# 236088/reflect-sampling-nerf

Hardware: AMD Instinct MI355X
Metric: rays/sec (train step) at 4096 rays x 128 samples, 1/2/4/8 MI355X; PSNR vs ref (higher is better)
Workload: dtype f32

## Files before the change

### reflect_sampling_nerf_amd/csrc/rsn_epilogues.h

```cpp
#pragma once
#include "rsn_gemm_loops.h"

template <int NBO>
__device__ __forceinline__ void init_acc(f32x16 (&acc)[NBO], const float* __restrict__ bias, int h) {
#pragma unroll
  for (int nb = 0; nb < NBO; ++nb)
#pragma unroll
    for (int q = 0; q < 4; ++q) {
      const float4 bv = *reinterpret_cast<const float4*>(bias + nb * 32 + 8 * q + 4 * h);
      acc[nb][4 * q + 0] = bv.x;
      acc[nb][4 * q + 1] = bv.y;
      acc[nb][4 * q + 2] = bv.z;
      acc[nb][4 * q + 3] = bv.w;
    }
}

template <int NBO>
__device__ __forceinline__ void zero_acc(f32x16 (&acc)[NBO]) {
#pragma unroll
  for (int nb = 0; nb < NBO; ++nb)
#pragma unroll
    for (int r = 0; r < 16; ++r) acc[nb][r] = 0.0f;
}

template <int NBO>
__device__ __forceinline__ void zero_acc16(f32x4 (&acc)[NBO][2][2]) {
#pragma unroll
  for (int nb = 0; nb < NBO; ++nb)
#pragma unroll
    for (int q = 0; q < 4; ++q) acc[nb][q >> 1][q & 1] = f32x4{0.0f, 0.0f, 0.0f, 0.0f};
}

template <int Q>
__device__ __forceinline__ unsigned relu_bits4q(unsigned b, const float4 v) {
  const unsigned lo[4] = {__float_as_uint(v.x), __float_as_uint(v.y), __float_as_uint(v.z), __float_as_uint(v.w)};
#pragma unroll
  for (int t = 0; t < 4; ++t) {
    unsigned bit, nb;
    if (Q == 0 && t == 0) {
      asm("v_min_u32 %0, %1, 1" : "=v"(bit) : "v"(lo[t]));
      b = bit;
    } else if (t == 0) {
      asm("v_min_u32 %0, %2, 1\n\tv_lshl_or_b32 %1, %0, %3, %4" : "=&v"(bit), "=v"(nb) : "v"(lo[t]), "n"(4 * Q), "v"(b));
      b = nb;
    } else if (t == 1) {
      asm("v_min_u32 %0, %2, 1\n\tv_lshl_or_b32 %1, %0, %3, %4" : "=&v"(bit), "=v"(nb) : "v"(lo[t]), "n"(4 * Q + 1), "v"(b));
      b = nb;
    } else if (t == 2) {
      asm("v_min_u32 %0, %2, 1\n\tv_lshl_or_b32 %1, %0, %3, %4" : "=&v"(bit), "=v"(nb) : "v"(lo[t]), "n"(4 * Q + 2), "v"(b));
      b = nb;
    } else {
      asm("v_min_u32 %0, %2, 1\n\tv_lshl_or_b32 %1, %0, %3, %4" : "=&v"(bit), "=v"(nb) : "v"(lo[t]), "n"(4 * Q + 3), "v"(b));
      b = nb;
    }
  }
  return b;
}
__device__ __forceinline__ unsigned relu_bits4(unsigned b, const float4 v, int q) {
  return q == 0 ? relu_bits4q<0>(b, v) : (q == 1 ? relu_bits4q<1>(b, v) : (q == 2 ? relu_bits4q<2>(b, v) : relu_bits4q<3>(b, v)));
}

template <int NBO>
struct ReluBits {
  unsigned w[NBO / 2];
};

template <int NBO>
__device__ __forceinline__ ReluBits<NBO> load_relu_bits(const unsigned* __restrict__ bits) {
  ReluBits<NBO> m;
  if (NBO >= 8) {
#pragma unroll
    for (int w4 = 0; w4 < NBO / 8; ++w4) {
      const uint4 v = *reinterpret_cast<const uint4*>(bits + w4 * 4);
      m.w[w4 * 4 + 0] = v.x; m.w[w4 * 4 + 1] = v.y; m.w[w4 * 4 + 2] = v.z; m.w[w4 * 4 + 3] = v.w;
    }
  } else {
#pragma unroll
    for (int w = 0; w < NBO / 2; ++w) m.w[w] = bits[w];
  }
  return m;
}

__device__ __forceinline__ unsigned bit_mask(int word, int pos) {
  unsigned m;
  asm("v_bfe_i32 %0, %1, %2, 1" : "=v"(m) : "v"(word), "n"(pos));
  return m;
}

template <int NBO, bool SBF = false, class SV = float*>
__device__ __forceinline__ void store_masked_bits(const f32x16 (&acc)[NBO], float4* xl, const ReluBits<NBO>& m, int h,
                                                  SV save = nullptr) {
#pragma unroll
  for (int nb = 0; nb < NBO; ++nb)
#pragma unroll
    for (int q = 0; q < 4; ++q) {
      const int word = m.w[nb / 2];
      const int base = (nb & 1) * 16 + 4 * q;
      float4 v;
      v.x = __uint_as_float(__float_as_uint(acc[nb][4 * q + 0]) & bit_mask(word, base + 0));
      v.y = __uint_as_float(__float_as_uint(acc[nb][4 * q + 1]) & bit_mask(word, base + 1));
      v.z = __uint_as_float(__float_as_uint(acc[nb][4 * q + 2]) & bit_mask(word, base + 2));
      v.w = __uint_as_float(__float_as_uint(acc[nb][4 * q + 3]) & bit_mask(word, base + 3));
      xl[(nb * 4 + q) * 64] = v;
      if (sv_on(save)) sv_put<SBF>(save, nb, q, h, v);
    }
}

template <int NBO>
__device__ __forceinline__ void store_masked_bits16(const f32x4 (&acc)[NBO][2][2], float4* xl, const ReluBits<NBO> (&m)[2], int lane) {
  const Lane16 g = lane16(lane);
  float4* xs = xl - lane + g.ol + g.kh * 64;
#pragma unroll
  for (int ph = 0; ph < 2; ++ph)
#pragma unroll
    for (int nb = 0; nb < NBO; ++nb) {
      const int word = (int)(m[ph].w[nb / 2] >> (4 * g.kh));
#pragma unroll
      for (int rh = 0; rh < 2; ++rh) {
        const int base = (nb & 1) * 16 + 8 * rh;
        const f32x4& a = acc[nb][rh][ph];
        float4 v;
        v.x = __uint_as_float(__float_as_uint(a[0]) & bit_mask(word, base + 0));
        v.y = __uint_as_float(__float_as_uint(a[1]) & bit_mask(word, base + 1));
        v.z = __uint_as_float(__float_as_uint(a[2]) & bit_mask(word, base + 2));
        v.w = __uint_as_float(__float_as_uint(a[3]) & bit_mask(word, base + 3));
        xs[(nb * 4 + 2 * rh) * 64 + 16 * ph] = v;
      }
    }
}

template <int NBO>
__device__ __forceinline__ void store_act16(const f32x4 (&acc)[NBO][2][2], float4* xl, int lane) {
  const Lane16 g = lane16(lane);
  float4* xs = xl - lane + g.ol + g.kh * 64;
#pragma unroll
  for (int nb = 0; nb < NBO; ++nb)
#pragma unroll
    for (int q = 0; q < 4; ++q) {
      const f32x4& a = acc[nb][q >> 1][q & 1];
      xs[(nb * 4 + 2 * (q >> 1)) * 64 + 16 * (q & 1)] = make_float4(a[0], a[1], a[2], a[3]);
    }
}

template <int NBS, bool RELU, bool SBF, bool REINIT, class ACC, class SV>
__device__ __forceinline__ void store_act_body(ACC& acc, float4* xl, SV save, int h, const float* __restrict__ bias, unsigned* bits) {
  unsigned bw[NBS / 2 > 0 ? NBS / 2 : 1];
#pragma unroll
  for (int nb = 0; nb < NBS; ++nb) {
    unsigned b16 = 0u;
#pragma unroll
    for (int q = 0; q < 4; ++q) {
      float4 v = make_float4(acc[nb][4 * q + 0], acc[nb][4 * q + 1], acc[nb][4 * q + 2], acc[nb][4 * q + 3]);
      if (RELU) {
        v.x = relu_f(v.x);
        v.y = relu_f(v.y);
        v.z = relu_f(v.z);
        v.w = relu_f(v.w);
        b16 = relu_bits4(b16, v, q);
      }
      xl[(nb * 4 + q) * 64] = v;
      if (sv_on(save)) sv_put<SBF>(save, nb, q, h, v);
      if constexpr (REINIT) {
        const float4 bv = *reinterpret_cast<const float4*>(bias + nb * 32 + 8 * q + 4 * h);
        acc[nb][4 * q + 0] = bv.x;
        acc[nb][4 * q + 1] = bv.y;
        acc[nb][4 * q + 2] = bv.z;
        acc[nb][4 * q + 3] = bv.w;
      }
    }
    if (RELU) {
      if (nb & 1) bw[nb / 2] |= b16 << 16; else bw[nb / 2] = b16;
    }
  }
  if (RELU && bits) {
    if (NBS >= 8) {
#pragma unroll
      for (int w4 = 0; w4 < NBS / 8; ++w4)
        *reinterpret_cast<uint4*>(bits + w4 * 4) = make_uint4(bw[w4 * 4], bw[w4 * 4 + 1], bw[w4 * 4 + 2], bw[w4 * 4 + 3]);
    } else {
#pragma unroll
      for (int w = 0; w < NBS / 2; ++w) bits[w] = bw[w];
    }
  }
}
template <int NBO, int NBS, bool RELU, bool SBF = false, class SV = float*>
__device__ __forceinline__ void store_act(const f32x16 (&acc)[NBO], float4* xl, SV save = nullptr, int h = 0,
                                          unsigned* bits = nullptr) {
  store_act_body<NBS, RELU, SBF, false>(acc, xl, save, h, nullptr, bits);
}
template <int NBO, bool RELU, bool SBF = false, class SV = float*>
__device__ __forceinline__ void store_act_init(f32x16 (&acc)[NBO], float4* xl, SV save, int h,
                                               const float* __restrict__ bias, unsigned* bits = nullptr) {
  store_act_body<NBO, RELU, SBF, true>(acc, xl, save, h, bias, bits);
}
```

### reflect_sampling_nerf_amd/csrc/rsn_field_kernel.h

```cpp
#pragma once
#include "rsn_epilogues.h"
#include "rsn_field_common.h"

template <int MODE, int NBO>
__device__ __forceinline__ void sweep_gemm(f32x16 (&acc)[NBO], const float* __restrict__ w32, const float* __restrict__ w16,
                                           const float4* xl, int n_it, int lane) {
  gemm_mode<MODE, NBO, NBO, true>(acc, w32, w16, xl, n_it, lane);
}
template <bool PACKED, int N_IT, int NBO>
__device__ __forceinline__ void sweep_gemm(f32x4 (&acc)[NBO][2][2], const float* __restrict__ w32, const float* __restrict__ w16,
                                           const float4* xl, int lane) {
  static_assert(N_IT % 4 == 0, "K = 8 N_IT is a multiple of 32 at every width (the units are padded to 32): no tail path");
  if constexpr (PACKED) gemm_bf16_s16<NBO>(acc, w16, xl, N_IT / 4, lane); else gemm_f32_x9_s16<NBO>(acc, w32, xl, N_IT / 4, lane);
}

template <int NB, bool TRAIN, int MMA>
__global__ __launch_bounds__(256) void rsn_field_kernel(const FieldJobs J) {
  using M = MmaTraits<MMA>;
  constexpr bool FOLD = M::FOLD;
  constexpr int MODE = M::LOOPS;
  static_assert(!FOLD || TRAIN, "the folded bottleneck serves the exact-fp32 training kernels");
  constexpr int NBH = FOLD ? 5 : NB + 1;
  constexpr int XITS = (NB * 4 > 16) ? NB * 4 : 16;
  constexpr int WAVE_F4 = (XITS + RSN_AUX_ITS) * 64;
  constexpr int W = NB * 32;
  constexpr bool SBF = TRAIN && M::SAVE_BF16;
  __shared__ float4 smem[4 * WAVE_F4];

  const int lane = threadIdx.x & 63;
  const int wid = __builtin_amdgcn_readfirstlane(threadIdx.x >> 6);
  float4* X = smem + wid * WAVE_F4 + lane;
  float4* AUX = X + XITS * 64;
  float* Xf = reinterpret_cast<float*>(X);

  const FieldShared& P = J.s;
  const TileJobs T = tile_space<128>(J);
  const float* __restrict__ pk = P.packed;

  for (long long gtile = blockIdx.x; gtile < T.n_tiles; gtile += gridDim.x) {
    const TileAt ta = tile_at(T, gtile);
    const FieldJob& a = J.j[ta.job];
    const long long n_points = ta.n_points, tile = ta.tile;
    const long long p0 = tile * 128 + wid * 32;
    if (p0 >= n_points) continue;
    int ln = lane;
    asm volatile("" : "+v"(ln));
    const int m = ln & 31, h = ln >> 5;
    const long long p = p0 + m;
    const bool valid = p < n_points;
    const long long pc = valid ? p : n_points - 1;
    const int rows = (int)(n_points - p0 < 32 ? n_points - p0 : 32);
    constexpr bool LOOPST = TRAIN && M::LOOP_STORES;
    auto rb_epi = [&](float* base, long long elem, int row_elems) {
      return rowbuf<SBF>((TRAIN && !LOOPST) ? base : nullptr, elem, rows, row_elems, m, h);
    };
    auto rb_loop = [&](float* base, long long elem, int row_elems) {
      return rowbuf<false>(LOOPST ? base : nullptr, elem, rows, row_elems, m, h);
    };
    auto bits_at = [&](int l) -> unsigned* {
      return a.saved.relu_bits + ((((long long)l * (a.act_stride / W)) + pc) * 2 + h) * (NB / 2 > 2 ? NB / 2 : 2);
    };

    float mc[3] = {0.0f, 0.0f, 0.0f}, vc[3] = {0.0f, 0.0f, 0.0f}, vd[3] = {0.0f, 0.0f, 0.0f};
    bool has_cov = true, has_dir = true;
    float4 wbh[NBH];
    const float* __restrict__ w_bh = pk + (FOLD ? P.L.w_fold : P.L.w_bh);
    if (a.mode == RSN_MODE_EMB) {
      pre_mode<MODE, NBH>(wbh, w_bh, ln);
      has_dir = a.view_dirs != nullptr;
#pragma unroll
      for (int c = 0; c < 3; ++c) vd[c] = has_dir ? a.view_dirs[pc * 3 + c] : 0.0f;
#pragma unroll 4
      for (int it = 0; it < NB * 4; ++it)
        X[it * 64] = *reinterpret_cast<const float4*>(a.emb_in + pc * W + it * 8 + 4 * h);
    } else {
    if (a.mode == RSN_MODE_FRUSTUM || a.mode == RSN_MODE_INF) {
      has_dir = point_gaussian(a, pc, mc, vc, vd);
    } else {
      has_cov = a.cov_diag != nullptr;
      has_dir = a.view_dirs != nullptr;
#pragma unroll
      for (int c = 0; c < 3; ++c) {
        mc[c] = a.means[pc * 3 + c];
        vc[c] = has_cov ? a.cov_diag[pc * 3 + c] : 0.0f;
        vd[c] = has_dir ? a.view_dirs[pc * 3 + c] : 0.0f;
      }
    }

#pragma unroll 1
    for (int c = 0; c < 3; ++c) {
      const float x = (c == 0) ? mc[0] : (c == 1 ? mc[1] : mc[2]);
      const float v = (c == 0) ? vc[0] : (c == 1 ? vc[1] : vc[2]);
      const float sx = 6.283185307179586f * x;
#pragma unroll 2
      for (int jj = 0; jj < 8; ++jj) {
        const float f = h ? P.freqs[8 + jj] : P.freqs[jj];
        const float ang = sx * f;
        const float e = has_cov ? expf(-0.5f * (v * (f * f))) : 1.0f;
        const float fs = e * sin_big(ang);
        const float fc = e * sin_big(ang + 1.5707963267948966f);
        const int u = c * 8 + jj;
        Xf[(u >> 2) * 256 + (u & 3)] = fs;
        Xf[((u + 24) >> 2) * 256 + ((u + 24) & 3)] = fc;
      }
    }
    {
      float4 raw = make_float4(0.0f, 0.0f, 0.0f, 0.0f);
      if (h == 0) raw = make_float4(mc[0], mc[1], mc[2], 0.0f);
      X[12 * 64] = raw;
      if (!M::F32) X[13 * 64] = make_float4(0.0f, 0.0f, 0.0f, 0.0f);
    }
    f32x16 st0, st1, st2;
    float4 st3;
    {
#pragma unroll
      for (int it = 0; it < 4; ++it) {
        const float4 t0 = X[it * 64], t1 = X[(4 + it) * 64], t2 = X[(8 + it) * 64];
        st0[4 * it + 0] = t0.x; st0[4 * it + 1] = t0.y; st0[4 * it + 2] = t0.z; st0[4 * it + 3] = t0.w;
        st1[4 * it + 0] = t1.x; st1[4 * it + 1] = t1.y; st1[4 * it + 2] = t1.z; st1[4 * it + 3] = t1.w;
        st2[4 * it + 0] = t2.x; st2[4 * it + 1] = t2.y; st2[4 * it + 2] = t2.z; st2[4 * it + 3] = t2.w;
      }
      st3 = X[12 * 64];
    }
    if (TRAIN && a.saved.enc && valid) {
      float* row = a.saved.enc + pc * RSN_K_ENC_PAD;
#pragma unroll
      for (int it = 0; it < RSN_ENC_ITS; ++it) *reinterpret_cast<float4*>(row + it * 8 + 4 * h) = X[it * 64];
    }

    {
      f32x16 acc[NB];
      float4 wpre[NB];
      pre_mode<MODE, NB>(wpre, pk + P.L.w_enc0, ln);
      init_acc<NB>(acc, pk + P.L.b[0], h);
      gemm_mode_run<MODE, NB, NB, TRAIN>(acc, wpre, pk + P.L.w_enc0, pk + P.L.h_enc0, X, RSN_ENC_ITS, ln);
#pragma unroll 1
      for (int l = 1; l < P.num_layers; ++l) {
        pre_mode<MODE, NB>(wpre, pk + P.L.w_x[l], ln);
        store_act_init<NB, true, SBF>(acc, X, rb_epi(a.saved.act, (l - 1) * a.act_stride + p0 * W, W),
                                 h, pk + P.L.b[l], (TRAIN && a.saved.relu_bits && valid) ? bits_at(l - 1) : nullptr);
        gemm_mode_run<MODE, NB, NB, TRAIN>(acc, wpre, pk + P.L.w_x[l], pk + P.L.h_x[l], X, NB * 4, ln,
                                rb_loop(a.saved.act, (l - 1) * a.act_stride + p0 * W, W));
        if (l == P.skip_layer) {
          pre_mode<MODE, NB>(wpre, pk + P.L.w_enc_skip, ln);
#pragma unroll
          for (int it = 0; it < 4; ++it) {
            X[it * 64] = make_float4(st0[4 * it], st0[4 * it + 1], st0[4 * it + 2], st0[4 * it + 3]);
            X[(4 + it) * 64] = make_float4(st1[4 * it], st1[4 * it + 1], st1[4 * it + 2], st1[4 * it + 3]);
            X[(8 + it) * 64] = make_float4(st2[4 * it], st2[4 * it + 1], st2[4 * it + 2], st2[4 * it + 3]);
          }
          X[12 * 64] = st3;
          if (!M::F32) X[13 * 64] = make_float4(0.0f, 0.0f, 0.0f, 0.0f);
          gemm_mode_run<MODE, NB, NB, TRAIN>(acc, wpre, pk + P.L.w_enc_skip, pk + P.L.h_enc_skip, X, RSN_ENC_ITS, ln);
        }
      }
      pre_mode<MODE, NBH>(wbh, w_bh, ln);
      store_act<NB, NB, true, SBF>(acc, X, rb_epi(a.saved.act, (P.num_layers - 1) * a.act_stride + p0 * W, W), h,
                              (TRAIN && a.saved.relu_bits && valid) ? bits_at(P.num_layers - 1) : nullptr);
    }
    }
    if (a.embedding && valid) {
#pragma unroll 4
      for (int it = 0; it < NB * 4; ++it)
        *reinterpret_cast<float4*>(a.embedding + pc * W + it * 8 + 4 * h) = X[it * 64];
    }

    float dcol[3], tcol[3], rho;
    float4 wmid[4];
    f32x16 accm[4];
    {
      f32x16 acc[NBH];
      init_acc<NBH>(acc, pk + (FOLD ? P.L.b_fold : P.L.b_bh), h);
      gemm_mode_run<MODE, NBH, NBH, TRAIN>(acc, wbh, w_bh, pk + P.L.h_bh, X, NB * 4, ln,
                                  rb_loop(a.mode == RSN_MODE_EMB ? nullptr : a.saved.act, (P.num_layers - 1) * a.act_stride + p0 * W, W));
      pre_mode<MODE, 4>(wmid, pk + P.L.w_mid_sh, ln);
      const float r0 = acc[NBH - 1][0], r1 = acc[NBH - 1][1], r2 = acc[NBH - 1][2], r3 = acc[NBH - 1][3];
      const float r4 = acc[NBH - 1][4], r5 = acc[NBH - 1][5], r6 = acc[NBH - 1][6];
      const float rough_raw = __shfl(r4, m, 64);
      rho = (a.mode == RSN_MODE_EMB && a.rough_in) ? a.rough_in[pc] : softplus_f(rough_raw);
      dcol[0] = sigmoid_f(r0); dcol[1] = sigmoid_f(r1); dcol[2] = sigmoid_f(r2);
      tcol[0] = sigmoid_f(r4); tcol[1] = sigmoid_f(r5); tcol[2] = sigmoid_f(r6);
      if (valid) {
        head_outputs_row<false, false>(h == 0 ? 0 : 1, a, P.density_bias, pc, make_float4(r0, r1, r2, r3), dcol, vd);
        head_outputs_row<false, false>(h == 0 ? 2 : 3, a, P.density_bias, pc, make_float4(r4, r5, r6, 0.0f), tcol, vd);
        if (TRAIN && a.saved.heads && h == 0) *reinterpret_cast<float4*>(a.saved.heads + pc * 8) = make_float4(r1, r2, r3, r4);
      }
      if constexpr (FOLD) {
#pragma unroll
        for (int nb = 0; nb < 4; ++nb) accm[nb] = acc[nb];
      } else {
        store_act<NBH, NB, false, SBF>(acc, X, rb_epi(a.saved.bott, p0 * W, W), h);
      }
    }

    {
      float sh[34];
      if (has_dir) {
        sh34_attenuated(vd[0], vd[1], vd[2], rho, sh);
      } else {
#pragma unroll
        for (int i = 0; i < 34; ++i) sh[i] = 0.0f;
      }
#pragma unroll
      for (int it = 0; it < RSN_SH_ITS; ++it) {
        float vals[4];
#pragma unroll
        for (int s = 0; s < 4; ++s) {
          const int u = it * 4 + s;
          vals[s] = (u < 17) ? (h ? sh[17 + u] : sh[u]) : 0.0f;
        }
        AUX[it * 64] = make_float4(vals[0], vals[1], vals[2], vals[3]);
        if (!M::F32 && it == 0) AUX[5 * 64] = make_float4(0.0f, 0.0f, 0.0f, 0.0f);
        if (TRAIN && a.saved.sh && valid)
          *reinterpret_cast<float4*>(a.saved.sh + pc * RSN_K_SH_PAD + it * 8 + 4 * h) =
              make_float4(vals[0], vals[1], vals[2], vals[3]);
      }
    }

    float4 wrgb[1];
    {
      if constexpr (FOLD) {
        gemm_mode_run<MODE, 4, 4, TRAIN>(accm, wmid, pk + P.L.w_mid_sh, pk + P.L.h_mid_sh, AUX, RSN_SH_ITS, ln);
      } else {
        init_acc<4>(accm, pk + P.L.b_mid, h);
        float4 wmx[4];
        pre_mode<MODE, 4>(wmx, pk + P.L.w_mid_x, ln);
        gemm_mode_run<MODE, 4, 4, TRAIN>(accm, wmid, pk + P.L.w_mid_sh, pk + P.L.h_mid_sh, AUX, RSN_SH_ITS, ln);
        gemm_mode_run<MODE, 4, 4, TRAIN>(accm, wmx, pk + P.L.w_mid_x, pk + P.L.h_mid_x, X, NB * 4, ln, rb_loop(a.saved.bott, p0 * W, W));
      }
      pre_mode<MODE, 1>(wrgb, pk + P.L.w_rgb, ln);
      store_act<4, 4, true, SBF>(accm, X, rb_epi(a.saved.hid, p0 * 128, 128), h,
                            (TRAIN && a.saved.relu_bits && valid) ? bits_at(P.num_layers) : nullptr);
    }
    {
      f32x16 accr[1];
      init_acc<1>(accr, pk + P.L.b_rgb, h);
      gemm_mode_run<MODE, 1, 1, TRAIN>(accr, wrgb, pk + P.L.w_rgb, pk + P.L.h_rgb, X, 16, ln, rb_loop(a.saved.hid, p0 * 128, 128));
      if (h == 1 && valid) colour_out<false, TRAIN>(a, pc, accr[0][0], accr[0][1], accr[0][2], dcol, tcol);
    }

    constexpr bool SEED_BITS = TRAIN && M::F32;
    if (TRAIN && a.saved.normals && a.saved.relu_bits) {
      const float* __restrict__ wd = pk + P.L.v_density;
      const bool peel = SEED_BITS && P.num_layers >= 2;
      if (peel) {
        const ReluBits<NB> m7 = load_relu_bits<NB>(bits_at(P.num_layers - 1));
        const ReluBits<NB> mb = load_relu_bits<NB>(bits_at(P.num_layers - 2));
        __builtin_amdgcn_sched_barrier(0);
        f32x16 acc[NB];
        zero_acc<NB>(acc);
        if constexpr (FOLD) {
          gemm_bf16_bits<NB>(acc, pk + P.L.hT_seed, m7, ln);
        } else {
          gemm_f32_bits<NB>(acc, pk + P.L.wT_x[P.num_layers - 1], wd, m7, ln);
        }
        store_masked_bits<NB>(acc, X, mb, h);
      } else {
        const ReluBits<NB> mb = load_relu_bits<NB>(bits_at(P.num_layers - 1));
#pragma unroll
        for (int it = 0; it < NB * 4; ++it) {
          const float4 w = *reinterpret_cast<const float4*>(wd + it * 8 + 4 * h);
          const int word = mb.w[it / 8];
          const int base = ((it / 4) & 1) * 16 + 4 * (it & 3);
          X[it * 64] = make_float4(
              __uint_as_float(__float_as_uint(w.x) & bit_mask(word, base + 0)),
              __uint_as_float(__float_as_uint(w.y) & bit_mask(word, base + 1)),
              __uint_as_float(__float_as_uint(w.z) & bit_mask(word, base + 2)),
              __uint_as_float(__float_as_uint(w.w) & bit_mask(word, base + 3)));
        }
      }
      if constexpr (SEED_BITS) {
        auto bits16_at = [&](int l, int ph) -> const unsigned* {
          const long long q = p0 + (ln & 15) + 16 * ph, qc = q < n_points ? q : n_points - 1;
          return a.saved.relu_bits + ((((long long)l * (a.act_stride / W)) + qc) * 2 + ((ln >> 4) & 1)) * (NB / 2 > 2 ? NB / 2 : 2);
        };
        f32x4 eacc[4][2][2];
        zero_acc16<4>(eacc);
#pragma unroll 1
        for (int l = P.num_layers - (peel ? 2 : 1); l >= 1; --l) {
          if (l == P.skip_layer) sweep_gemm<FOLD, NB * 4, 4>(eacc, pk + P.L.wT_enc_skip, pk + P.L.hT_enc_skip, X, ln);
          const ReluBits<NB> mb[2] = {load_relu_bits<NB>(bits16_at(l - 1, 0)), load_relu_bits<NB>(bits16_at(l - 1, 1))};
          __builtin_amdgcn_sched_barrier(0);
          f32x4 acc[NB][2][2];
// ... 54 lines not shown
```

### reflect_sampling_nerf_amd/csrc/rsn_gemm_loops.h

```cpp
#pragma once
#include "rsn_device_math.h"

template <bool SBF>
__device__ __forceinline__ void put4(float* save, int off, const float4 v) {
  if (SBF) {
    const bf16x4 o = {(__bf16)v.x, (__bf16)v.y, (__bf16)v.z, (__bf16)v.w};
    *reinterpret_cast<bf16x4*>(reinterpret_cast<__bf16*>(save) + off) = o;
  } else {
    *reinterpret_cast<float4*>(save + off) = v;
  }
}

#define RSN_SAVED_ROW_AUX 0
struct RowBuf {
  __amdgpu_buffer_rsrc_t r;
  unsigned voff;
  unsigned lim;
  bool on;
};
template <bool SBF>
__device__ __forceinline__ RowBuf rowbuf(float* base, long long elem, int rows, int row_elems, int m, int h) {
  constexpr int BPE = SBF ? 2 : 4;
  RowBuf b;
  b.on = !(__builtin_constant_p(base == nullptr) && base == nullptr);
// ... 376 lines not shown
    c = __builtin_amdgcn_mfma_f32_32x32x16_bf16(s3, b, c, 0, 0, 0);
    c = __builtin_amdgcn_mfma_f32_32x32x16_bf16(s2, b, c, 0, 0, 0);
    c = __builtin_amdgcn_mfma_f32_32x32x16_bf16(s1, b, c, 0, 0, 0);
    acc[nb0 + t] = c;
  }
}

template <int NBO, class BITS>
__device__ __forceinline__ void gemm_f32_bits(f32x16 (&acc)[NBO], const float* __restrict__ w32seg, const float* __restrict__ wd,
                                              const BITS& m, int lane) {
  static_assert(NBO % 2 == 0, "two fragment buffers of NBO / 2 blocks");
  constexpr int NH = NBO / 2, NK = 2 * NBO;
  const WBuf wp = wbuf_make(w32seg, lane);
  const float* __restrict__ wdl = wd + 4 * (lane >> 5);
  float4 fa[NH][2], fb[NH][2];
  load_w32_pair<NBO, NH>(fa, wp, 0, 0);
  const SeedWords mw = seed_words<NBO>(m);
  float4 dlo = *reinterpret_cast<const float4*>(wdl), dhi = *reinterpret_cast<const float4*>(wdl + 8);
#pragma unroll 1
  for (int kk = 0; kk < NK; ++kk) {
    load_w32_pair<NBO, NH>(fb, wp, kk, NH);
    const int kn = (kk + 1 < NK) ? kk + 1 : kk;
    const float4 nlo = *reinterpret_cast<const float4*>(wdl + 16 * kn), nhi = *reinterpret_cast<const float4*>(wdl + 16 * kn + 8);
    const bf16x8 bc = bits_bf16x8(mw, kk);
    mma16_bits_f32<NBO, NH>(acc, fa, dlo, dhi, bc, 0);
    __builtin_amdgcn_sched_barrier(0);
    load_w32_pair<NBO, NH>(fa, wp, kn, 0);
    mma16_bits_f32<NBO, NH>(acc, fb, dlo, dhi, bc, NH);
    __builtin_amdgcn_sched_barrier(0);
    dlo = nlo; dhi = nhi;
  }
}

struct Lane16 {
  int ol;
  int kh;
};
__device__ __forceinline__ Lane16 lane16(int lane) {
  Lane16 g;
  g.ol = (lane & 15) + 2 * (lane & 16);
  g.kh = lane >> 5;
  return g;
}

__device__ __forceinline__ bf16x8 piece(const BSplit& b, int k) { return k == 0 ? b.s1 : (k == 1 ? b.s2 : b.s3); }
constexpr int x9_wp(int p) { constexpr int t[9] = {2, 2, 1, 2, 1, 0, 1, 0, 0}; return t[p]; }
constexpr int x9_bp(int p) { constexpr int t[9] = {2, 1, 2, 0, 1, 2, 0, 1, 0}; return t[p]; }
template <int NBO, int NQ>
__device__ __forceinline__ void mma16s(f32x4 (&acc)[NBO][2][2], const bf16x8 (&w)[NQ][2][3], const BSplit (&b)[2], int nb0) {
#pragma unroll
  for (int t = 0; t < NQ; ++t)
#pragma unroll
    for (int p = 0; p < 9; ++p)
#pragma unroll
      for (int q = 0; q < 4; ++q)
        acc[nb0 + t][q >> 1][q & 1] = __builtin_amdgcn_mfma_f32_16x16x32_bf16(w[t][q >> 1][x9_wp(p)], piece(b[q & 1], x9_bp(p)),
                                                                              acc[nb0 + t][q >> 1][q & 1], 0, 0, 0);
}

template <int NQ>
__device__ __forceinline__ void load_w16s(bf16x8 (&w)[NQ][2][3], const WBuf& wp, int s, int nbo, int nb0) {
#pragma unroll
  for (int t = 0; t < NQ; ++t)
#pragma unroll
    for (int rh = 0; rh < 2; ++rh)
#pragma unroll
      for (int sp = 0; sp < 3; ++sp) {
        const u32x4 v = __builtin_amdgcn_raw_buffer_load_b128(wp.r, wp.voff + rh * 256u, (unsigned)(((2 * s * nbo + nb0 + t) * 3 + sp) * 1024), 0);
        w[t][rh][sp] = __builtin_bit_cast(bf16x8, v);
      }
}

__device__ __forceinline__ void sv_put16(const float*, int, int, bool, const float4, const float4) {}
__device__ __forceinline__ void sv_put16(const RowBuf& b, int it, int ph, bool live, const float4 lo, const float4 hi) {
  const unsigned at = b.voff + (unsigned)ph * 16u * b.lim + (unsigned)it * 32u;
  const unsigned o0 = (live && (unsigned)it * 32u < b.lim) ? at : 0x80000000u;
  const unsigned o1 = (live && (unsigned)it * 32u + 32u < b.lim) ? at + 32u : 0x80000000u;
  const u32x4 v0 = {__float_as_uint(lo.x), __float_as_uint(lo.y), __float_as_uint(lo.z), __float_as_uint(lo.w)};
  const u32x4 v1 = {__float_as_uint(hi.x), __float_as_uint(hi.y), __float_as_uint(hi.z), __float_as_uint(hi.w)};
  __builtin_amdgcn_raw_buffer_store_b128(v0, b.r, o0, 0, RSN_SAVED_ROW_AUX);
  __builtin_amdgcn_raw_buffer_store_b128(v1, b.r, o1, 0, RSN_SAVED_ROW_AUX);
}

template <int NBO, class SV = const float*>
__device__ __forceinline__ void gemm_bf16_s16(f32x4 (&acc)[NBO][2][2], const float* __restrict__ wseg, const float4* xl, int n_k32,
                                              int lane, SV save = nullptr) {
  static_assert(NBO % 2 == 0, "an even number of fragment buffers' worth of blocks");
  constexpr int NQ = NBO >= 4 ? NBO / 4 : 1, NC = NBO / NQ;
  const Lane16 g = lane16(lane);
  WBuf wp = wbuf_make(wseg, lane);
  wp.voff = (unsigned)g.ol * 16u + (unsigned)g.kh * (NBO * 3072u);
  const float4* xb = xl - lane + g.ol + g.kh * 128;
  bf16x8 wa[NQ][2][3], wb[NQ][2][3];
  load_w16s<NQ>(wa, wp, 0, NBO, 0);
  BSplit bc[2];
  if (sv_on(save)) {
    const float4 p0lo = xb[0], p0hi = xb[64], p1lo = xb[16], p1hi = xb[80];
    bc[0] = split8<3>(p0lo, p0hi);
    bc[1] = split8<3>(p1lo, p1hi);
    sv_put16(save, 2 * g.kh, 0, true, p0lo, p0hi);
    sv_put16(save, 2 * g.kh, 1, true, p1lo, p1hi);
  } else {
    bc[0] = split8<3>(xb[0], xb[64]);
    bc[1] = split8<3>(xb[16], xb[80]);
  }
  const int s1 = n_k32 > 1 ? 1 : 0;
  float4 x0lo = xb[4 * s1 * 64], x0hi = xb[(4 * s1 + 1) * 64], x1lo = xb[4 * s1 * 64 + 16], x1hi = xb[(4 * s1 + 1) * 64 + 16];
#pragma unroll 1
  for (int s = 0; s < n_k32; ++s) {
    const int sn = (s + 1 < n_k32) ? s + 1 : s;
    const int s2 = (s + 2 < n_k32) ? s + 2 : sn;
    BSplit bn[2];
#pragma unroll
    for (int c = 0; c < NC; ++c) {
      if (c & 1) load_w16s<NQ>(wa, wp, c + 1 < NC ? s : sn, NBO, c + 1 < NC ? (c + 1) * NQ : 0);
      else load_w16s<NQ>(wb, wp, s, NBO, (c + 1) * NQ);
      __builtin_amdgcn_sched_barrier(0);
      if (c == 0) bn[0] = split8<3>(x0lo, x0hi);
      if (c == 1) bn[1] = split8<3>(x1lo, x1hi);
      if (c == 0 && sv_on(save)) sv_put16(save, 4 * sn + 2 * g.kh, 0, s + 1 < n_k32, x0lo, x0hi);
      if (c == 1 && sv_on(save)) sv_put16(save, 4 * sn + 2 * g.kh, 1, s + 1 < n_k32, x1lo, x1hi);
      if (c == NC - 1) {
        x0lo = xb[4 * s2 * 64]; x0hi = xb[(4 * s2 + 1) * 64];
        x1lo = xb[4 * s2 * 64 + 16]; x1hi = xb[(4 * s2 + 1) * 64 + 16];
      }
      if (c & 1) mma16s<NBO, NQ>(acc, wb, bc, c * NQ); else mma16s<NBO, NQ>(acc, wa, bc, c * NQ);
#pragma unroll
      for (int m = 0; m < NQ * 36; ++m) {
        __builtin_amdgcn_sched_group_barrier(0x008, 1, 0);
        if (c < 2) __builtin_amdgcn_sched_group_barrier(0x002, 2, 0);
        if (c < 2 && sv_on(save) && (m == 8 || m == 20)) __builtin_amdgcn_sched_group_barrier(0x040, 1, 0);
      }
      if (c == NC - 1) __builtin_amdgcn_sched_group_barrier(0x100, 4, 0);
      __builtin_amdgcn_sched_barrier(0);
    }
    bc[0] = bn[0];
    bc[1] = bn[1];
  }
}

template <int NQ>
__device__ __forceinline__ void load_w32s(float4 (&f)[NQ][2][2], const WBuf& b, int s, int nbo, int nb0) {
#pragma unroll
  for (int t = 0; t < NQ; ++t)
#pragma unroll
    for (int rh = 0; rh < 2; ++rh)
#pragma unroll
      for (int j = 0; j < 2; ++j) {
        const u32x4 v = __builtin_amdgcn_raw_buffer_load_b128(b.r, b.voff + rh * 256u, (unsigned)(((4 * s + j) * nbo + nb0 + t) * 1024), 0);
        f[t][rh][j] = make_float4(__uint_as_float(v.x), __uint_as_float(v.y), __uint_as_float(v.z), __uint_as_float(v.w));
      }
}

template <int NBO>
__device__ __forceinline__ void gemm_f32_x9_s16(f32x4 (&acc)[NBO][2][2], const float* __restrict__ w32seg, const float4* xl,
                                                int n_k32, int lane) {
  static_assert(NBO % 2 == 0, "an even number of fragment buffers' worth of blocks");
  constexpr int NQ = NBO >= 4 ? NBO / 4 : 1, NC = NBO / NQ, UQ = 2 * NQ, NU = 2 * NBO;
  const Lane16 g = lane16(lane);
  WBuf wp = wbuf_make(w32seg, lane);
  wp.voff = (unsigned)g.ol * 16u + (unsigned)g.kh * (NBO * 2048u);
  const float4* xb = xl - lane + g.ol + g.kh * 128;
  float4 fa[NQ][2][2], fb[NQ][2][2];
  load_w32s<NQ>(fa, wp, 0, NBO, 0);
  load_w32s<NQ>(fb, wp, 0, NBO, NQ);
  BSplit bc[2] = {split8<3>(xb[0], xb[64]), split8<3>(xb[16], xb[80])};
  const int s1 = n_k32 > 1 ? 1 : 0;
  float4 x0lo = xb[4 * s1 * 64], x0hi = xb[(4 * s1 + 1) * 64], x1lo = xb[4 * s1 * 64 + 16], x1hi = xb[(4 * s1 + 1) * 64 + 16];
  BSplit w = split8<3>(fa[0][0][0], fa[0][0][1]);
  BSplit bn[2] = {bc[0], bc[1]};
#pragma unroll 1
  for (int s = 0; s < n_k32; ++s) {
    const int sn = (s + 1 < n_k32) ? s + 1 : s;
    const int s2 = (s + 2 < n_k32) ? s + 2 : sn;
#pragma unroll
    for (int u = 0; u < NU; ++u) {
      const int un = (u + 1) % NU, cn = (un / UQ) & 1, tn = (un / 2) % NQ;
      const BSplit wn = cn ? split8<3>(fb[tn][un & 1][0], fb[tn][un & 1][1]) : split8<3>(fa[tn][un & 1][0], fa[tn][un & 1][1]);
      const bool reload = u % UQ == UQ - 1;
      if (reload) {
        const int c = u / UQ, c2 = (c + 2) % NC;
        if (c & 1) load_w32s<NQ>(fb, wp, c + 2 < NC ? s : sn, NBO, c2 * NQ);
        else load_w32s<NQ>(fa, wp, c + 2 < NC ? s : sn, NBO, c2 * NQ);
      }
      if (u == NU - 2) bn[0] = split8<3>(x0lo, x0hi);
      if (u == NU - 1) {
        bn[1] = split8<3>(x1lo, x1hi);
        x0lo = xb[4 * s2 * 64]; x0hi = xb[(4 * s2 + 1) * 64];
        x1lo = xb[4 * s2 * 64 + 16]; x1hi = xb[(4 * s2 + 1) * 64 + 16];
      }
#pragma unroll
      for (int p = 0; p < 9; ++p)
#pragma unroll
        for (int ph = 0; ph < 2; ++ph)
          acc[u >> 1][u & 1][ph] = __builtin_amdgcn_mfma_f32_16x16x32_bf16(piece(w, x9_wp(p)), piece(bc[ph], x9_bp(p)),
                                                                           acc[u >> 1][u & 1][ph], 0, 0, 0);
#pragma unroll
      for (int m = 0; m < 18; ++m) {
        __builtin_amdgcn_sched_group_barrier(0x008, 1, 0);
        if (reload && m < NQ * 4) __builtin_amdgcn_sched_group_barrier(0x020, 1, 0);
        if (u >= NU - 2) __builtin_amdgcn_sched_group_barrier(0x002, 6, 0);
        else __builtin_amdgcn_sched_group_barrier(0x002, 3, 0);
      }
      if (u == NU - 1) __builtin_amdgcn_sched_group_barrier(0x100, 4, 0);
      __builtin_amdgcn_sched_barrier(0);
      w = wn;
    }
    bc[0] = bn[0];
    bc[1] = bn[1];
  }
}
```

### reflect_sampling_nerf_amd/csrc/rsn_pack.hip

```cpp
#include <stdarg.h>
#include <stdlib.h>
#include <string.h>

#include <string>
#include <vector>

#include "rsn_common.h"

static thread_local std::string g_last_error;

void rsn_set_error(const char* fmt, ...) {
  char buf[1024];
  va_list ap;
  va_start(ap, fmt);
  vsnprintf(buf, sizeof(buf), fmt, ap);
  va_end(ap);
  g_last_error = buf;
}

extern "C" const char* rsn_last_error(void) { return g_last_error.c_str(); }

int rsn_device_cus() {
  static int cache[64] = {0};
  int dev = 0;
// ... 394 lines not shown
  return j;
}

int job_blocks(const PackJob& j) {
  return ((j.is_bias ? j.n_rows : j.n_it * j.nbo * (j.layout >= 1 ? 512 : 256)) + 255) / 256;
}
int split_blocks(const SplitSeg& s) { return (((s.n_it + 1) / 2) * s.nbo * 512 + 255) / 256; }

int build_jobs(const rsn_field_desc* d, const rsn_field_params* p, float* packed, const RsnPackedLayout& L,
               std::vector<PackJob>& jobs, std::vector<SplitSeg>& splits) {
  const int WP = d->width, W = (d->param_width > 0 ? d->param_width : d->width), MW = d->mid_width, NB = L.nb, NBM = L.nbm;
  const int n_layers = d->num_layers, skip = d->skip_layer, mid_in = RSN_SH_DIM + W;
  auto in_f = [&](int l) { return l == 0 ? RSN_ENC_DIM : (l == skip ? RSN_ENC_DIM + W : W); };
  auto x_off = [&](int l) { return l == skip ? RSN_ENC_DIM : 0; };
  auto gemm = [&](const float* w, int ld, size_t dst, int n_it, int nbo, int transpose = 0) {
    PackJob* j = add_job(jobs);
    j->src[0] = w; j->ld[0] = ld; j->dst = packed + dst; j->n_it = n_it; j->nbo = nbo; j->transpose = transpose;
    return j;
  };
  auto bias = [&](const float* b, size_t dst, int n_rows) {
    PackJob* j = add_job(jobs);
    j->is_bias = 1; j->src[0] = b; j->dst = packed + dst; j->n_rows = n_rows;
    return j;
  };
  PackJob* j;
  for (int l = 0; l < n_layers; ++l) {
    RSN_REQUIRE(p->trunk_w[l] && p->trunk_b[l], RSN_ERR_INVALID_ARGUMENT, "trunk layer %d has NULL parameters", l);
    if (l >= 1) {
      j = gemm(p->trunk_w[l], in_f(l), L.w_x[l], NB * 4, NB);
      rows_natural(*j, W); cols_natural(*j, W, x_off(l));
    }
    if (l == 0 || l == skip) {
      j = gemm(p->trunk_w[l], in_f(l), l == 0 ? L.w_enc0 : L.w_enc_skip, RSN_ENC_ITS, NB);
      rows_natural(*j, W); cols_slots(*j, RSN_K_ENC_PAD, enc_slot_to_column);
    }
    rows_natural(*bias(p->trunk_b[l], L.b[l], WP), W);
  }

  RSN_REQUIRE(p->density_w && p->normals_w && p->roughness_w && p->diff_w && p->tint_w && p->bottleneck_w &&
                  p->mid_w && p->rgb_w && p->density_b && p->normals_b && p->roughness_b && p->diff_b &&
                  p->tint_b && p->bottleneck_b && p->mid_b && p->rgb_b,
              RSN_ERR_INVALID_ARGUMENT, "a head parameter pointer is NULL");
  const float* const heads_w[5] = {p->density_w, p->normals_w, p->diff_w, p->roughness_w, p->tint_w};
  const float* const heads_b[5] = {p->density_b, p->normals_b, p->diff_b, p->roughness_b, p->tint_b};

  j = gemm(p->bottleneck_w, W, L.w_bh, NB * 4, NB + 1);
  heads_src(*j, 1, heads_w, W); rows_natural(*j, W); heads_rows(*j, WP); cols_natural(*j, W, 0);
  j = bias(p->bottleneck_b, L.b_bh, WP + 32);
  heads_src(*j, 1, heads_b, 0); rows_natural(*j, W); heads_rows(*j, WP);
  j = gemm(p->mid_w, mid_in, L.w_mid_sh, RSN_SH_ITS, NBM);
  rows_natural(*j, MW); cols_slots(*j, RSN_K_SH_PAD, sh_slot_to_column);
  j = gemm(p->mid_w, mid_in, L.w_mid_x, NB * 4, NBM);
  rows_natural(*j, MW); cols_natural(*j, W, RSN_SH_DIM);
  rows_natural(*bias(p->mid_b, L.b_mid, MW), MW);
  j = gemm(p->rgb_w, MW, L.w_rgb, NBM * 4, 1);
  rows_rgb(*j); cols_natural(*j, MW, 0);
  rows_rgb(*bias(p->rgb_b, L.b_rgb, 32));

  for (int l = 1; l < n_layers; ++l) {
    j = gemm(p->trunk_w[l], in_f(l), L.wT_x[l], NB * 4, NB, 1);
    rows_natural(*j, W, x_off(l)); cols_natural(*j, W, 0);
  }
  for (int l : {0, skip}) {
    if (l < 0) continue;
    j = gemm(p->trunk_w[l], in_f(l), l == 0 ? L.wT_enc0 : L.wT_enc_skip, NB * 4, 4, 1);
    rows_from(*j, 128, enc_slot_to_column); cols_natural(*j, W, 0);
  }
  j = gemm(p->bottleneck_w, W, L.wT_bh, NB * 4, NB, 1);
  rows_natural(*j, W); cols_natural(*j, W, 0);
  j = gemm(nullptr, 0, L.wT_bh + (size_t)(NB * 4) * NB * 256, 4, NB, 3);
  heads_src(*j, 0, heads_w, W); rows_natural(*j, W); cols_headsT(*j, false);
  j = gemm(p->mid_w, mid_in, L.wT_mid_x, NBM * 4, NB, 1);
  rows_natural(*j, W, RSN_SH_DIM); cols_natural(*j, MW, 0);
  j = gemm(p->rgb_w, MW, L.wT_rgb, 4, NBM, 1);
  rows_natural(*j, MW);
  for (int c = 0; c < 3; ++c) j->col[4 + c] = (int16_t)c;
  rows_natural(*bias(p->density_w, L.v_density, WP), W);

  if (L.q_stream != 0) {
    int frag = 0;
    auto ring = [&](const float* w, int ld, int ks, int nbo16, int transpose = 0) {
      PackJob* q = gemm(w, ld, L.q_stream + (size_t)frag * 256 * L.q_pf, ks, nbo16, transpose);
      q->layout = L.q_pf == 3 ? 2 : 1;
      frag += ks * nbo16;
      return q;
    };
    for (int l = 0; l < n_layers; ++l) {
      if (l >= 1) {
        j = ring(p->trunk_w[l], in_f(l), 8, 16);
        rows_perm16(*j, WP, W); cols_natural(*j, W, x_off(l));
      }
      if (l == 0 || l == skip) {
        j = ring(p->trunk_w[l], in_f(l), 4, 16);
        rows_perm16(*j, WP, W); cols_slots(*j, 128, enc16_slot_to_column);
      }
    }
    j = ring(nullptr, W, 8, 2);
    heads_src(*j, 1, heads_w, W); heads_rows(*j, 0); cols_natural(*j, W, 0);
    j = ring(p->bottleneck_w, W, 8, 16);
    rows_perm16(*j, WP, W); cols_natural(*j, W, 0);
    j = ring(p->mid_w, mid_in, 2, 8);
    rows_perm16(*j, MW, MW); cols_slots(*j, 64, sh16_slot_to_column);
    j = ring(p->mid_w, mid_in, 8, 8);
    rows_perm16(*j, MW, MW); cols_natural(*j, W, RSN_SH_DIM);
    j = ring(p->rgb_w, MW, 4, 4);
    rows_rgb(*j); cols_natural(*j, MW, 0);
    RSN_REQUIRE(frag * L.q_pf == L.q_groups * 16, RSN_ERR_INVALID_ARGUMENT, "16x32 stream: %d fragments, layout says %d groups",
                frag, L.q_groups);
    j = ring(p->rgb_w, MW, 2, 8, 1);
    rows_perm16(*j, MW, MW);
    for (int c = 0; c < 3; ++c) j->col[8 + c] = (int16_t)c;
    j = ring(p->mid_w, mid_in, 4, 16, 1);
    rows_perm16(*j, WP, W, RSN_SH_DIM); cols_natural(*j, MW, 0);
    j = ring(p->bottleneck_w, W, 8, 16, 1);
    rows_perm16(*j, WP, W); cols_natural(*j, W, 0);
    j = ring(nullptr, 0, 1, 16, 3);
    heads_src(*j, 0, heads_w, W); rows_perm16(*j, WP, W); cols_headsT(*j, true);
    for (int l = n_layers - 1; l >= 0; --l) {
      if (l == 0 || l == skip) {
        j = ring(p->trunk_w[l], in_f(l), 8, 8, 1);
        rows_from(*j, 128, [](int n) { return enc16_slot_to_column(perm16_row_to_feature(n)); }); cols_natural(*j, W, 0);
      }
      if (l >= 1) {
        j = ring(p->trunk_w[l], in_f(l), 8, 16, 1);
        rows_perm16(*j, WP, W, x_off(l)); cols_natural(*j, W, 0);
      }
    }
    RSN_REQUIRE(frag * L.q_pf == L.t_g_end * 16, RSN_ERR_INVALID_ARGUMENT, "transposed 16x32 stream: %d fragments, layout says %d groups",
                frag, L.t_g_end);
  }

  if (d->mma_mode == RSN_MMA_F32_FOLDED) {
    const float* wc = packed + L.fold_wc;
    j = gemm(wc, W, L.w_fold, NB * 4, NBM + 1);
    heads_src(*j, 1, heads_w, W); rows_natural(*j, MW); heads_rows(*j, MW); cols_natural(*j, W, 0);
    j = bias(packed + L.fold_bc, L.b_fold, MW + 32);
    heads_src(*j, 1, heads_b, 0); rows_natural(*j, MW); heads_rows(*j, MW);
    j = gemm(wc, W, L.wT_fold, NBM * 4, NB, 1);
    rows_natural(*j, W); cols_natural(*j, MW, 0);
    j = gemm(nullptr, 0, L.wT_fold + (size_t)(NBM * 4) * NB * 256, 4, NB, 3);
    heads_src(*j, 0, heads_w, W); rows_natural(*j, W); cols_headsT(*j, false);
  }

  auto split = [&](size_t src, int n_it, int nbo, size_t dst, size_t kscale = 0) {
    splits.push_back(SplitSeg{(unsigned)src, (unsigned)dst, (short)n_it, (short)nbo, 0, (unsigned)kscale});
  };
  if (d->mma_mode == RSN_MMA_F32 || d->mma_mode == RSN_MMA_F32_FOLDED) {
    if (L.hT_seed != 0) split(L.wT_x[n_layers - 1], NB * 4, NB, L.hT_seed, L.v_density);
    if (d->mma_mode == RSN_MMA_F32_FOLDED) {
      for (int l = 1; l + 1 < n_layers; ++l) split(L.wT_x[l], NB * 4, NB, L.hT_x[l]);
      if (L.hT_last != 0) split(L.wT_x[n_layers - 1], NB * 4, NB, L.hT_last);
      if (skip >= 1) split(L.wT_enc_skip, NB * 4, 4, L.hT_enc_skip);
      split(L.wT_enc0, NB * 4, 4, L.hT_enc0);
    }
    return RSN_OK;
  }
  split(L.w_enc0, RSN_ENC_ITS, NB, L.h_enc0);
  for (int l = 1; l < n_layers; ++l) {
    split(L.w_x[l], NB * 4, NB, L.h_x[l]);
    split(L.wT_x[l], NB * 4, NB, L.hT_x[l]);
  }
  if (skip >= 1) {
    split(L.w_enc_skip, RSN_ENC_ITS, NB, L.h_enc_skip);
    split(L.wT_enc_skip, NB * 4, 4, L.hT_enc_skip);
  }
  split(L.wT_enc0, NB * 4, 4, L.hT_enc0);
  split(L.w_bh, NB * 4, NB + 1, L.h_bh);
  split(L.wT_bh, NB * 4 + 4, NB, L.hT_bh);
  split(L.w_mid_sh, RSN_SH_ITS, NBM, L.h_mid_sh);
  split(L.w_mid_x, NB * 4, NBM, L.h_mid_x);
  split(L.wT_mid_x, NBM * 4, NB, L.hT_mid_x);
  split(L.w_rgb, NBM * 4, 1, L.h_rgb);
  split(L.wT_rgb, 4, NBM, L.hT_rgb);
  return RSN_OK;
}

thread_local std::vector<PackJob> t_jobs;
thread_local std::vector<SplitSeg> t_splits;

int validate_and_build(const rsn_field_desc* d, const rsn_field_params* p, float* packed, size_t packed_bytes) {
  RsnPackedLayout L;
  const int rc = rsn_compute_layout(d, &L);
  if (rc != RSN_OK) return rc;
  RSN_REQUIRE(p != nullptr && packed != nullptr, RSN_ERR_INVALID_ARGUMENT, "params/packed is NULL");
  RSN_REQUIRE(packed_bytes >= L.total * sizeof(float), RSN_ERR_WORKSPACE,
              "packed buffer too small: %zu < %zu bytes", packed_bytes, L.total * sizeof(float));
  t_jobs.clear(); t_splits.clear();
  return build_jobs(d, p, packed, L, t_jobs, t_splits);
}

}

static int launch_fold(const rsn_field_desc* d, const rsn_field_params* p, float* packed, hipStream_t st) {
  if (d->mma_mode != RSN_MMA_F32_FOLDED) return RSN_OK;
  RsnPackedLayout L;
  RSN_TRY(rsn_compute_layout(d, &L));
  const int w = d->param_width > 0 ? d->param_width : d->width, n = d->mid_width * w + d->mid_width;
  hipLaunchKernelGGL(rsn_fold_kernel, dim3((unsigned)((n + 255) / 256)), dim3(256), 0, st, p->mid_w, p->mid_b, p->bottleneck_w,
                     p->bottleneck_b, w, d->mid_width, packed + L.fold_wc, packed + L.fold_bc);
  RSN_HIP(hipGetLastError());
  return RSN_OK;
}

extern "C" int rsn_pack_weights(const rsn_field_desc* d, const rsn_field_params* p, float* packed,
                                size_t packed_bytes, void* stream) {
  const int rc = validate_and_build(d, p, packed, packed_bytes);
  if (rc != RSN_OK) return rc;
  hipStream_t st = (hipStream_t)stream;
  RSN_TRY(launch_fold(d, p, packed, st));
  for (const PackJob& j : t_jobs) {
    hipLaunchKernelGGL(rsn_pack_kernel, dim3((unsigned)job_blocks(j)), dim3(256), 0, st, j);
    RSN_HIP(hipGetLastError());
  }
  for (const SplitSeg& s : t_splits) {
    hipLaunchKernelGGL(rsn_pack_split_kernel, dim3((unsigned)split_blocks(s)), dim3(256), 0, st, packed + s.src, (int)s.n_it,
                       (int)s.nbo, packed + s.dst, s.kscale ? packed + s.kscale : nullptr);
    RSN_HIP(hipGetLastError());
  }
  return RSN_OK;
}

extern "C" size_t rsn_pack_table_bytes(void) { return sizeof(PackTable); }

extern "C" int rsn_pack_weights_table(const rsn_field_desc* d, const rsn_field_params* p, float* packed,
                                      size_t packed_bytes, void* table, size_t table_bytes, int32_t rebuild_table,
                                      void* stream) {
  RSN_REQUIRE(table != nullptr && table_bytes >= sizeof(PackTable), RSN_ERR_WORKSPACE,
              "job table buffer too small: %zu < %zu bytes", table_bytes, sizeof(PackTable));
  const int rc = validate_and_build(d, p, packed, packed_bytes);
  if (rc != RSN_OK) return rc;
  RSN_REQUIRE((int)t_jobs.size() <= PACK_MAX_JOBS && (int)t_splits.size() <= SPLIT_MAX_SEGS, RSN_ERR_UNSUPPORTED,
              "%zu pack jobs / %zu split segments exceed the table", t_jobs.size(), t_splits.size());
  hipStream_t st = (hipStream_t)stream;
  static thread_local PackTable host_table;
  const int n_jobs = (int)t_jobs.size();
  int blocks = 0;
  for (int i = 0; i < n_jobs; ++i) {
    if (rebuild_table) { host_table.block_start[i] = blocks; host_table.jobs[i] = t_jobs[i]; }
    blocks += job_blocks(t_jobs[i]);
  }
  if (rebuild_table) {
    host_table.n_jobs = n_jobs;
    host_table.n_blocks = host_table.block_start[n_jobs] = blocks;
    RSN_HIP(hipMemcpyAsync(table, &host_table, sizeof(PackTable), hipMemcpyHostToDevice, st));
  }
  RSN_TRY(launch_fold(d, p, packed, st));
  hipLaunchKernelGGL(rsn_pack_all_kernel, dim3((unsigned)blocks), dim3(256), 0, st, (const PackTable*)table);
  RSN_HIP(hipGetLastError());
  if (!t_splits.empty()) {
    SplitJob sj;
    memset(&sj, 0, sizeof(sj));
    sj.packed = packed; sj.n_segs = (int)t_splits.size();
    int b = 0;
    for (int i = 0; i < sj.n_segs; ++i) {
      sj.s[i] = t_splits[i];
      sj.s[i].block0 = b;
      b += split_blocks(sj.s[i]);
    }
    hipLaunchKernelGGL(rsn_pack_split_all_kernel, dim3((unsigned)b), dim3(256), 0, st, sj);
    RSN_HIP(hipGetLastError());
  }
  return RSN_OK;
}
```

Measured before the change: 99310.

## Route f32 training trunk layers through 16x16 MFMA sweep with fused activation save

```diff
diff --git a/reflect_sampling_nerf_amd/csrc/rsn_epilogues.h b/reflect_sampling_nerf_amd/csrc/rsn_epilogues.h
--- a/reflect_sampling_nerf_amd/csrc/rsn_epilogues.h
+++ b/reflect_sampling_nerf_amd/csrc/rsn_epilogues.h
@@ -142,6 +142,90 @@
     }
 }
 
+template <int NBO>
+__device__ __forceinline__ void init_acc16(f32x4 (&acc)[NBO][2][2], const float* __restrict__ bias, int lane) {
+  const float* __restrict__ bl = bias + 4 * (lane >> 4);
+#pragma unroll
+  for (int nb = 0; nb < NBO; ++nb)
+#pragma unroll
+    for (int rh = 0; rh < 2; ++rh) {
+      const float4 bv = *reinterpret_cast<const float4*>(bl + nb * 32 + 16 * rh);
+      acc[nb][rh][0] = acc[nb][rh][1] = f32x4{bv.x, bv.y, bv.z, bv.w};
+    }
+}
+
+template <int NBO, bool REINIT>
+__device__ __forceinline__ void store_act16_relu_body(f32x4 (&acc)[NBO][2][2], float4* xl, int lane, const float* __restrict__ bias,
+                                                      unsigned* bits) {
+  static_assert(NBO % 2 == 0, "whole mask words");
+  const Lane16 g = lane16(lane);
+  float4* xs = xl - lane + g.ol + g.kh * 64;
+  const float* __restrict__ bl = bias + 4 * (lane >> 4);
+  unsigned bw[2][NBO / 2];
+#pragma unroll
+  for (int nb = 0; nb < NBO; ++nb) {
+    unsigned b16[2] = {0u, 0u};
+#pragma unroll
+    for (int rh = 0; rh < 2; ++rh) {
+#pragma unroll
+      for (int ph = 0; ph < 2; ++ph) {
+        const f32x4& a = acc[nb][rh][ph];
+        const float4 v = make_float4(relu_f(a[0]), relu_f(a[1]), relu_f(a[2]), relu_f(a[3]));
+        b16[ph] = relu_bits4(b16[ph], v, 2 * rh);
+        xs[(nb * 4 + 2 * rh) * 64 + 16 * ph] = v;
+      }
+      if constexpr (REINIT) {
+        const float4 bv = *reinterpret_cast<const float4*>(bl + nb * 32 + 16 * rh);
+        acc[nb][rh][0] = acc[nb][rh][1] = f32x4{bv.x, bv.y, bv.z, bv.w};
+      }
+    }
+#pragma unroll
+    for (int ph = 0; ph < 2; ++ph) {
+      if (nb & 1) bw[ph][nb / 2] |= b16[ph] << 16; else bw[ph][nb / 2] = b16[ph];
+    }
+  }
+  unsigned ow[NBO / 2];
+#pragma unroll
+  for (int w = 0; w < NBO / 2; ++w) {
+    const unsigned keep = (g.kh ? bw[1][w] : bw[0][w]) << (4 * g.kh);
+    const unsigned give = (g.kh ? bw[0][w] : bw[1][w]) << (4 * g.kh);
+    ow[w] = keep | (unsigned)__shfl_xor((int)give, 32, 64);
+  }
+  if (bits) {
+    if (NBO >= 8) {
+#pragma unroll
+      for (int w4 = 0; w4 < NBO / 8; ++w4)
+        *reinterpret_cast<uint4*>(bits + w4 * 4) = make_uint4(ow[w4 * 4], ow[w4 * 4 + 1], ow[w4 * 4 + 2], ow[w4 * 4 + 3]);
+    } else {
+#pragma unroll
+      for (int w = 0; w < NBO / 2; ++w) bits[w] = ow[w];
+    }
+  }
+}
+template <int NBO>
+__device__ __forceinline__ void store_act16_relu(f32x4 (&acc)[NBO][2][2], float4* xl, int lane, unsigned* bits) {
+  store_act16_relu_body<NBO, false>(acc, xl, lane, nullptr, bits);
+}
+template <int NBO>
+__device__ __forceinline__ void store_act16_relu_init(f32x4 (&acc)[NBO][2][2], float4* xl, int lane, const float* __restrict__ bias,
+                                                      unsigned* bits) {
+  store_act16_relu_body<NBO, true>(acc, xl, lane, bias, bits);
+}
+
+template <int NBO>
+__device__ __forceinline__ void load_acc(f32x16 (&acc)[NBO], const float4* xl) {
+#pragma unroll
+  for (int nb = 0; nb < NBO; ++nb)
+#pragma unroll
+    for (int q = 0; q < 4; ++q) {
+      const float4 v = xl[(nb * 4 + q) * 64];
+      acc[nb][4 * q + 0] = v.x;
+      acc[nb][4 * q + 1] = v.y;
+      acc[nb][4 * q + 2] = v.z;
+      acc[nb][4 * q + 3] = v.w;
+    }
+}
+
 template <int NBS, bool RELU, bool SBF, bool REINIT, class ACC, class SV>
 __device__ __forceinline__ void store_act_body(ACC& acc, float4* xl, SV save, int h, const float* __restrict__ bias, unsigned* bits) {
   unsigned bw[NBS / 2 > 0 ? NBS / 2 : 1];
diff --git a/reflect_sampling_nerf_amd/csrc/rsn_field_kernel.h b/reflect_sampling_nerf_amd/csrc/rsn_field_kernel.h
--- a/reflect_sampling_nerf_amd/csrc/rsn_field_kernel.h
+++ b/reflect_sampling_nerf_amd/csrc/rsn_field_kernel.h
@@ -7,11 +7,12 @@
                                            const float4* xl, int n_it, int lane) {
   gemm_mode<MODE, NBO, NBO, true>(acc, w32, w16, xl, n_it, lane);
 }
-template <bool PACKED, int N_IT, int NBO>
+template <bool PACKED, int N_IT, int NBO, class SV = const float*>
 __device__ __forceinline__ void sweep_gemm(f32x4 (&acc)[NBO][2][2], const float* __restrict__ w32, const float* __restrict__ w16,
-                                           const float4* xl, int lane) {
+                                           const float4* xl, int lane, SV save = nullptr) {
   static_assert(N_IT % 4 == 0, "K = 8 N_IT is a multiple of 32 at every width (the units are padded to 32): no tail path");
-  if constexpr (PACKED) gemm_bf16_s16<NBO>(acc, w16, xl, N_IT / 4, lane); else gemm_f32_x9_s16<NBO>(acc, w32, xl, N_IT / 4, lane);
+  if constexpr (PACKED) gemm_bf16_s16<NBO>(acc, w16, xl, N_IT / 4, lane, save);
+  else gemm_f32_x9_s16<NBO>(acc, w32, xl, N_IT / 4, lane, save);
 }
 
 template <int NB, bool TRAIN, int MMA>
@@ -128,7 +129,63 @@
       for (int it = 0; it < RSN_ENC_ITS; ++it) *reinterpret_cast<float4*>(row + it * 8 + 4 * h) = X[it * 64];
     }
 
-    {
+    bool s16 = false;
+    if constexpr (TRAIN && M::F32) s16 = a.mode == RSN_MODE_FRUSTUM || a.mode == RSN_MODE_INF;
+    if (s16) {
+     if constexpr (TRAIN && M::F32) {
+      auto bits16_st = [&](int l) -> unsigned* {
+        const long long q = p0 + (ln & 15) + 16 * (ln >> 5);
+        if (!a.saved.relu_bits || q >= n_points) return nullptr;
+        return a.saved.relu_bits + ((((long long)l * (a.act_stride / W)) + q) * 2 + ((ln >> 4) & 1)) * (NB / 2 > 2 ? NB / 2 : 2);
+      };
+      auto rb_loop16 = [&](float* base, long long elem, int row_elems) {
+        return rowbuf<false>(base, elem, rows, row_elems, ln & 15, (ln >> 4) & 1);
+      };
+      {
+        f32x16 acc[NB];
+        float4 wpre[NB];
+        pre_mode<MODE, NB>(wpre, pk + P.L.w_enc0, ln);
+        init_acc<NB>(acc, pk + P.L.b[0], h);
+        gemm_mode_run<MODE, NB, NB, TRAIN>(acc, wpre, pk + P.L.w_enc0, pk + P.L.h_enc0, X, RSN_ENC_ITS, ln);
+        if (P.num_layers == 1) pre_mode<MODE, NBH>(wbh, w_bh, ln);
+        store_act<NB, NB, true, false>(acc, X, rb_epi(a.saved.act, p0 * W, W), h, (a.saved.relu_bits && valid) ? bits_at(0) : nullptr);
+      }
+      if (P.num_layers > 1) {
+        f32x4 a16[NB][2][2];
+        init_acc16<NB>(a16, pk + P.L.b[1], ln);
+#pragma unroll 1
+        for (int l = 1; l < P.num_layers; ++l) {
+          sweep_gemm<FOLD, NB * 4, NB>(a16, pk + P.L.w_x[l], pk + P.L.h_x[l], X, ln,
+                                       rb_loop16(a.saved.act, (l - 1) * a.act_stride + p0 * W, W));
+          const bool last = l + 1 == P.num_layers;
+          if (l == P.skip_layer) {
+            f32x16 acc[NB];
+            float4 wpre[NB];
+            pre_mode<MODE, NB>(wpre, pk + P.L.w_enc_skip, ln);
+            store_act16<NB>(a16, X, ln);
+            load_acc<NB>(acc, X);
+#pragma unroll
+            for (int it = 0; it < 4; ++it) {
+              X[it * 64] = make_float4(st0[4 * it], st0[4 * it + 1], st0[4 * it + 2], st0[4 * it + 3]);
+              X[(4 + it) * 64] = make_float4(st1[4 * it], st1[4 * it + 1], st1[4 * it + 2], st1[4 * it + 3]);
+              X[(8 + it) * 64] = make_float4(st2[4 * it], st2[4 * it + 1], st2[4 * it + 2], st2[4 * it + 3]);
+            }
+            X[12 * 64] = st3;
+            gemm_mode_run<MODE, NB, NB, TRAIN>(acc, wpre, pk + P.L.w_enc_skip, pk + P.L.h_enc_skip, X, RSN_ENC_ITS, ln);
+            if (last) pre_mode<MODE, NBH>(wbh, w_bh, ln);
+            store_act<NB, NB, true, false>(acc, X, rb_epi(a.saved.act, p0 * W, W), h,
+                                           (a.saved.relu_bits && valid) ? bits_at(l) : nullptr);
+            if (!last) init_acc16<NB>(a16, pk + P.L.b[l + 1], ln);
+          } else if (!last) {
+            store_act16_relu_init<NB>(a16, X, ln, pk + P.L.b[l + 1], bits16_st(l));
+          } else {
+            pre_mode<MODE, NBH>(wbh, w_bh, ln);
+            store_act16_relu<NB>(a16, X, ln, bits16_st(l));
+          }
+        }
+      }
+     }
+    } else {
       f32x16 acc[NB];
       float4 wpre[NB];
       pre_mode<MODE, NB>(wpre, pk + P.L.w_enc0, ln);
diff --git a/reflect_sampling_nerf_amd/csrc/rsn_gemm_loops.h b/reflect_sampling_nerf_amd/csrc/rsn_gemm_loops.h
--- a/reflect_sampling_nerf_amd/csrc/rsn_gemm_loops.h
+++ b/reflect_sampling_nerf_amd/csrc/rsn_gemm_loops.h
@@ -552,9 +552,9 @@
       }
 }
 
-template <int NBO>
+template <int NBO, class SV = const float*>
 __device__ __forceinline__ void gemm_f32_x9_s16(f32x4 (&acc)[NBO][2][2], const float* __restrict__ w32seg, const float4* xl,
-                                                int n_k32, int lane) {
+                                                int n_k32, int lane, SV save = nullptr) {
   static_assert(NBO % 2 == 0, "an even number of fragment buffers' worth of blocks");
   constexpr int NQ = NBO >= 4 ? NBO / 4 : 1, NC = NBO / NQ, UQ = 2 * NQ, NU = 2 * NBO;
   const Lane16 g = lane16(lane);
@@ -564,7 +564,17 @@
   float4 fa[NQ][2][2], fb[NQ][2][2];
   load_w32s<NQ>(fa, wp, 0, NBO, 0);
   load_w32s<NQ>(fb, wp, 0, NBO, NQ);
-  BSplit bc[2] = {split8<3>(xb[0], xb[64]), split8<3>(xb[16], xb[80])};
+  BSplit bc[2];
+  if (sv_on(save)) {
+    const float4 p0lo = xb[0], p0hi = xb[64], p1lo = xb[16], p1hi = xb[80];
+    bc[0] = split8<3>(p0lo, p0hi);
+    bc[1] = split8<3>(p1lo, p1hi);
+    sv_put16(save, 2 * g.kh, 0, true, p0lo, p0hi);
+    sv_put16(save, 2 * g.kh, 1, true, p1lo, p1hi);
+  } else {
+    bc[0] = split8<3>(xb[0], xb[64]);
+    bc[1] = split8<3>(xb[16], xb[80]);
+  }
   const int s1 = n_k32 > 1 ? 1 : 0;
   float4 x0lo = xb[4 * s1 * 64], x0hi = xb[(4 * s1 + 1) * 64], x1lo = xb[4 * s1 * 64 + 16], x1hi = xb[(4 * s1 + 1) * 64 + 16];
   BSplit w = split8<3>(fa[0][0][0], fa[0][0][1]);
@@ -584,6 +594,8 @@
         else load_w32s<NQ>(fa, wp, c + 2 < NC ? s : sn, NBO, c2 * NQ);
       }
       if (u == NU - 2) bn[0] = split8<3>(x0lo, x0hi);
+      if (u == NU - 2 && sv_on(save)) sv_put16(save, 4 * sn + 2 * g.kh, 0, s + 1 < n_k32, x0lo, x0hi);
+      if (u == NU - 1 && sv_on(save)) sv_put16(save, 4 * sn + 2 * g.kh, 1, s + 1 < n_k32, x1lo, x1hi);
       if (u == NU - 1) {
         bn[1] = split8<3>(x1lo, x1hi);
         x0lo = xb[4 * s2 * 64]; x0hi = xb[(4 * s2 + 1) * 64];
@@ -601,6 +613,7 @@
         if (reload && m < NQ * 4) __builtin_amdgcn_sched_group_barrier(0x020, 1, 0);
         if (u >= NU - 2) __builtin_amdgcn_sched_group_barrier(0x002, 6, 0);
         else __builtin_amdgcn_sched_group_barrier(0x002, 3, 0);
+        if (u >= NU - 2 && sv_on(save) && (m == 5 || m == 12)) __builtin_amdgcn_sched_group_barrier(0x040, 1, 0);
       }
       if (u == NU - 1) __builtin_amdgcn_sched_group_barrier(0x100, 4, 0);
       __builtin_amdgcn_sched_barrier(0);
diff --git a/reflect_sampling_nerf_amd/csrc/rsn_pack.hip b/reflect_sampling_nerf_amd/csrc/rsn_pack.hip
--- a/reflect_sampling_nerf_amd/csrc/rsn_pack.hip
+++ b/reflect_sampling_nerf_amd/csrc/rsn_pack.hip
@@ -570,6 +570,7 @@
       if (L.hT_last != 0) split(L.wT_x[n_layers - 1], NB * 4, NB, L.hT_last);
       if (skip >= 1) split(L.wT_enc_skip, NB * 4, 4, L.hT_enc_skip);
       split(L.wT_enc0, NB * 4, 4, L.hT_enc0);
+      for (int l = 1; l < n_layers; ++l) split(L.w_x[l], NB * 4, NB, L.h_x[l]);
     }
     return RSN_OK;
   }
```

New measurement: 101,700, median of 6. 1.02x the previous value.
